# nanoporetech/bonito

Hardware: AMD Instinct MI355X
Metric: signal samples/sec/GPU (chunk=10000, batch=512) + read accuracy vs ref (higher is better)
Workload: dtype f16

## Files before the change

### bonito_amd/_lib.py

```python
import ctypes as C
import os

_HERE = os.path.dirname(os.path.abspath(__file__))
LIB_PATH = os.environ.get("BONITO_HIP_LIB") or os.path.join(_HERE, "libbonito_hip.so")


class HipEngineError(RuntimeError):
    """An entry point of libbonito_hip.so reported an error."""


class bh_layer_t(C.Structure):
    _fields_ = [
        ("kind", C.c_int32), ("in_size", C.c_int32), ("out_size", C.c_int32),
        ("winlen", C.c_int32), ("stride", C.c_int32), ("padding", C.c_int32),
        ("activation", C.c_int32), ("reverse", C.c_int32),
        ("nhead", C.c_int32), ("dim_ff", C.c_int32), ("win_left", C.c_int32), ("win_right", C.c_int32),
        ("scale_factor", C.c_int32), ("groups", C.c_int32), ("add_residual", C.c_int32), ("quantize", C.c_int32), ("reserved_i", C.c_int32 * 1),
        ("scale", C.c_float), ("clamp_lo", C.c_float), ("clamp_hi", C.c_float),
        ("blank_score", C.c_float), ("alpha", C.c_float), ("eps", C.c_float), ("reserved_f", C.c_float * 2),
        ("w0", C.c_void_p), ("b0", C.c_void_p), ("w1", C.c_void_p), ("b1", C.c_void_p),
        ("w2", C.c_void_p), ("w3", C.c_void_p), ("w4", C.c_void_p), ("w5", C.c_void_p),
    ]


# ... 20 lines not shown
    "bh_encoder_ack": (_i, [_vp, _l]),
    "bh_encoder_describe": (_i, [_vp, C.c_char_p, _sz]),
    "bh_encoder_profile": (_i, [_vp, _i]),
    "bh_encoder_profile_read": (_i, [_vp, C.POINTER(C.c_float), C.POINTER(_i)]),
    "bh_crf_viterbi_workspace": (_sz, [_i, _i, _i]),
    "bh_crf_viterbi": (_i, [_vp, _i, _i, _i, _i, _f, _l, _l, _vp, _vp, _vp, _vp, _vp]),
    "bh_crf_reverse_complement": (_i, [_vp, _vp, _i, _i, _i, _i, _l, _l, _vp]),
    "bh_crf_logz": (_i, [_vp, _i, _i, _i, _f, _vp, _vp, _vp]),
    "bh_crf_seq_workspace": (_sz, [_i, _i, _i, _i]),
    "bh_crf_seq_logz": (_i, [_vp, _i, _i, _i, _i, _f, _l, _l, _vp, _i, _i, _vp, _vp, _vp, _vp]),
    "bh_crf_seq_viterbi": (_i, [_vp, _i, _i, _i, _i, _f, _l, _l, _vp, _i, _i, _vp, _vp, _vp, _vp, _vp]),
    "bh_crf_seq_logz_free": (_i, [_vp, _i, _i, _i, _f, _l, _l, _vp, _i, _i, _vp, _vp, _vp, _vp]),
    "bh_crf_logz_dense": (_i, [_vp, _i, _i, _i, _i, _f, _l, _l, _vp, _vp]),
    "bh_sw_workspace": (_sz, [_i, _i, _i]),
    "bh_sw_align": (_i, [_vp, _l, _vp, _vp, _l, _vp, _i, _i, _i, _i, _i, _vp, _sz, _vp, _vp, _l, _vp, _vp]),
    "bh_set_option": (_i, [C.c_char_p, _i]),
    "bh_signal_normalise": (_i, [_vp, _vp, _vp, _vp, _i, _i, C.c_double, C.c_double, C.c_double, C.c_double, C.c_double, C.c_double,
                            _i, _vp, _vp, _vp, _vp, _vp]),
    "bh_signal_chunks": (_i, [_vp, _vp, _vp, _vp, _vp, _vp, _vp, _vp, _vp, _vp, _i, _i, _vp, _vp]),
    "bh_crf_posterior_viterbi_workspace": (_sz, [_i, _i, _i]),
    "bh_crf_posterior_viterbi": (_i, [_vp, _i, _i, _i, _f, _vp, _vp, _vp, _vp]),
    "bh_beam_search_workspace": (_sz, [_i, _i, _i]),
    "bh_beam_search": (_i, [_vp, _i, _i, _i, _i, _f, _f, _f, _f, _vp, _vp, _vp, _vp, _vp, _vp]),
    "bh_linear": (_i, [_vp, _vp, _vp, _vp, _i, _i, _i, _i, _i, _i, _i, _f, _f, _f, _i, _i, _l, _l, _i, _vp]),
    "bh_conv1d_first": (_i, [_vp, _vp, _vp, _vp, _i, _i, _i, _i, _i, _i, _i, _f, _f, _l, _l, _vp]),
    "bh_conv1d_packed_halves": (_sz, [_i, _i, _i]),
    "bh_conv1d_pack": (_i, [_vp, _i, _i, _i, _vp]),
    "bh_conv1d": (_i, [_vp, _vp, _vp, _vp, _i, _i, _i, _i, _i, _i, _i, _i, _f, _f, _l, _l, _vp]),
    "bh_ctc_greedy_decode": (_i, [_vp, _vp, _i, _i, _f, _f, _vp, _vp, _vp, _vp, _vp]),
    "bh_ctc_beam_search_workspace": (_sz, [_l, _i, _i, _i]),
    "bh_ctc_beam_search": (_i, [_vp, _vp, _i, _i, _i, _f, _vp, _vp, _vp, _vp, _vp]),
    "bh_dwconv1d": (_i, [_vp, _vp, _vp, _i, _i, _i, _i, _i, _i, _vp]),
    "bh_rotary_table": (_i, [_i, _i, _vp]),
    "bh_attention": (_i, [_vp, _vp, _vp, _i, _i, _i, _i, _i, _i, _vp]),
    "bh_attention_prerotated": (_i, [_vp, _vp, _i, _i, _i, _i, _i, _i, _vp]),
    "bh_rmsnorm_residual": (_i, [_vp, _vp, _vp, _vp, _l, _i, _f, _f, _vp]),
    "bh_lstm_pack_whh": (_i, [_vp, _i, _vp]),
    "bh_host_compact": (_l, [_vp, _l, _vp]),
    "bh_host_chunk_rows": (_l, [_vp, _l, _i, _i, _l, _l, _vp]),
    "bh_host_format_read": (_l, [_vp, _vp, _vp, _vp, _i, _l, _l, _i, _i, _i, _i, _i, _i, C.c_double, C.c_char_p, C.c_char_p, _l, _l,
                                 _vp, _l, _vp, _vp]),
    "bh_host_mean_qscore": (C.c_double, [C.c_char_p, _l]),
    "bh_host_svb16_decode": (_l, [_vp, _l, _l, _vp]),
    "bh_lstm_workspace": (_sz, [_i, _i]),
    "bh_lstm_layer": (_i, [_vp, _vp, _vp, _i, _i, _i, _i, _vp, _vp, _i, _vp]),
    "bh_lstm_q8_layer": (_i, [_vp, _f, _vp, _vp, _vp, _i, _i, _i, _i, _i, _vp, _vp, _vp, _vp]),
# ... 47 lines not shown
```

### bonito_amd/csrc/beam.hip

```cpp
#include <stdlib.h>

#include "common.h"
#include "kernels.h"
#include <cstring>
#include "../../include/bh_lse_table.h"

namespace bh {

__device__ const float g_lse_tab[BH_LSE_TABLE_SIZE] = {BH_LSE_TABLE_VALUES};

__device__ __forceinline__ float lse2_tab(float a, float b, const float* tab) {
    float m = fmaxf(a, b);
    float d = fabsf(a - b);
    if (!(d < BH_LSE_RANGE)) return m;
    float x = d * BH_LSE_SCALE;
    int i = (int)x;
    float f = x - (float)i;
    float t0 = tab[i];
    float sp = __fmaf_rn(f, tab[i + 1] - t0, t0);
    return m + sp;
}

__device__ __forceinline__ float lse2_tab_nb(float a, float b, const float* tab) {
    const float m = fmaxf(a, b);
// ... 222 lines not shown
                res_m[t - tlo] = (int8_t)(k != 0);
                res_p[t - tlo] = (int8_t)(k != 0 ? 1 + (st & 3) : 0);
                if (k != 0) st = (k - 1) * q + (st >> 2);
            }
            s_state[0] = st;
        }
        __syncthreads();
        for (int i = threadIdx.x; i < thi - tlo; i += blockDim.x) { mo[tlo + i] = res_m[i]; pth[tlo + i] = res_p[i]; }
        __syncthreads();
    }
}

struct BeamArgs {
    const half_t* scores;
    const float* beta;
    int N, T, S, state_len, W;
    float blank, cut;
    uint8_t* bp;
    int* final_slot;
    long long* dbg;
    float inv_bin;
    float* P;
    int nt;
};

template <int STATE_LEN>
__host__ __device__ constexpr int beam_btb() {
#ifdef BH_BTB
    return BH_BTB;
#else
    return STATE_LEN >= 4 ? 1 : 2;
#endif
}
constexpr int MAXW = 32;

__device__ __forceinline__ unsigned bs_hash0(int s) { return ((unsigned)s + 1u) * 2654435761u; }
__device__ __forceinline__ unsigned bs_mix(unsigned h, int x) {
    h = (h ^ ((unsigned)x + 1u)) * 16777619u;
    return h ^ (h >> 15);
}
__device__ __forceinline__ unsigned bs_ukey(float k) {
    unsigned u = __float_as_uint(k);
    return (u & 0x80000000u) ? ~u : (u | 0x80000000u);
}
__device__ __forceinline__ int popc64(unsigned long long m) { return __popcll(m); }
__device__ __forceinline__ unsigned long long lanemask_lt(int lane) { return (1ull << lane) - 1ull; }
// ... 170 lines not shown
constexpr unsigned TAG_MASK = 0x1ffffu;

struct BeamTable {
    int* cnt;
    uint2_t* ent;
    int* ov_cnt;
    uint2_t* ov;
};

__device__ __forceinline__ unsigned bucket_match(const uint4_t& e0, unsigned hash, unsigned want) {
    unsigned d = 32u;
    d = min(d, e0.x == hash ? e0.y - want : 32u);
    d = min(d, e0.z == hash ? e0.w - want : 32u);
    return d;
}

__device__ __forceinline__ void dma16(const char* g, char* lds) {
    const unsigned l = (unsigned)__builtin_amdgcn_readfirstlane((int)(unsigned)(size_t)(__attribute__((address_space(3))) char*)lds);
    asm volatile("s_mov_b32 m0, %0\n\ts_nop 0\n\tglobal_load_lds_dwordx4 %1, off" ::"s"(l), "v"(g) : "memory");
}
__device__ __forceinline__ void dma16_nt(const char* g, char* lds) {
    const unsigned l = (unsigned)__builtin_amdgcn_readfirstlane((int)(unsigned)(size_t)(__attribute__((address_space(3))) char*)lds);
    asm volatile("s_mov_b32 m0, %0\n\ts_nop 0\n\tglobal_load_lds_dwordx4 %1, off nt" ::"s"(l), "v"(g) : "memory");
}

#include "../../include/bh_bs2.h"
typedef float float2_t __attribute__((ext_vector_type(2)));

__device__ __forceinline__ float2_t fma2(float2_t a, float2_t b, float2_t c) { return __builtin_elementwise_fma(a, b, c); }
__device__ __forceinline__ float2_t splat2(float v) { return float2_t{v, v}; }

__device__ __forceinline__ float2_t bs2_exp2(float2_t x) {
    x.x = __builtin_amdgcn_fmed3f(x.x, -BH_BS2_XMAX, BH_BS2_XMAX);
    x.y = __builtin_amdgcn_fmed3f(x.y, -BH_BS2_XMAX, BH_BS2_XMAX);
    const float2_t t = fma2(x, splat2(BH_BS2_LOG2E), splat2(BH_BS2_MAGIC));
    const float2_t n = t - splat2(BH_BS2_MAGIC);
    const float2_t f = fma2(x, splat2(BH_BS2_LOG2E), -n);
    float2_t p = splat2(BH_BS2_E5);
    p = fma2(p, f, splat2(BH_BS2_E4));
    p = fma2(p, f, splat2(BH_BS2_E3));
    p = fma2(p, f, splat2(BH_BS2_E2));
    p = fma2(p, f, splat2(BH_BS2_E1));
    p = fma2(p, f, splat2(BH_BS2_E0));
    float2_t r;
    r.x = __uint_as_float(__float_as_uint(p.x) + (__float_as_uint(t.x) << 23));
    r.y = __uint_as_float(__float_as_uint(p.y) + (__float_as_uint(t.y) << 23));
// ... 370 lines not shown
                    Pn[(long)t * 4 + m_raw] = (m_raw == 0 ? c4[0] : m_raw == 1 ? c4[1] : m_raw == 2 ? c4[2] : c4[3]) / tot;
                }
            } else {
                if (act) *(float4_t*)(an + 4 * m) = o;
                const float inv = 1.0f / ((cls[0] + cls[1]) + (cls[2] + cls[3]));
                if (lane < 4 && live) Pn[(long)t * 4 + lane] = (lane == 0 ? cls[0] : lane == 1 ? cls[1] : lane == 2 ? cls[2] : cls[3]) * inv;
            }
            cur ^= 1;
        }
    }
}

template <int STATE_LEN, int CPW, bool FUSE>
__host__ __device__ constexpr int beam_scan_waves() { return !FUSE ? 0 : (1 << (2 * STATE_LEN)) / 4 >= 64 ? CPW : 1; }

template <int STATE_LEN, int CPW, bool DBG, bool FUSE = false>
__global__ __launch_bounds__(64 * (CPW + beam_scan_waves<STATE_LEN, CPW, FUSE>())) __attribute__((amdgpu_waves_per_eu(1, 8))) void beam_kernel(BeamArgs p) {
    extern __shared__ __attribute__((aligned(16))) char smem[];
    constexpr int S = 1 << (2 * STATE_LEN);
    constexpr int sh = 2 * (STATE_LEN - 1);
    constexpr int BTB = beam_btb<STATE_LEN>();
    constexpr int QS = S / 4, GLS = QS < 64 ? QS : 64;
    constexpr int NTHR = 64 * (CPW + beam_scan_waves<STATE_LEN, CPW, FUSE>());
    static_assert(!FUSE || QS >= 64 || CPW * QS <= 64, "one scan wave must hold the chunks of the workgroup");
    static_assert(NBK == HBINS, "the selection histogram reuses the bucket fill counters");
    static_assert(beam_wave_lds<STATE_LEN>() % 16 == 0 && BEAM_TAB_LDS % 16 == 0, "LDS regions must stay 16-byte aligned");
    const int T = p.T, W = p.W;
    const int lane = threadIdx.x & 63;
    const int wave_all = __builtin_amdgcn_readfirstlane(threadIdx.x >> 6);
    const bool scan_role = FUSE && wave_all >= CPW;
    const int slot_raw = !scan_role ? wave_all : QS >= 64 ? wave_all - CPW : lane / GLS;
    const bool slot_ok = slot_raw < CPW && blockIdx.x * CPW + slot_raw < p.N;
    const int wave = slot_ok ? slot_raw : 0;
    const int n = blockIdx.x * CPW + wave;
    float* tab = (float*)smem;
    for (int i = threadIdx.x; i < BH_LSE_TABLE_SIZE; i += NTHR) tab[i] = g_lse_tab[i];
    __syncthreads();
    if (!slot_ok && (!scan_role || QS >= 64)) return;
    char* mine = smem + BEAM_TAB_LDS + wave * beam_wave_lds<STATE_LEN>();
    half_t* st_sc = (half_t*)mine;
    float* st_b = (float*)(st_sc + 2 * BTB * 4 * S);
    constexpr int SCAN_LDS = scan_wave_lds<STATE_LEN>();
    char* scan_mem = smem + BEAM_TAB_LDS + CPW * beam_wave_lds<STATE_LEN>() + wave * SCAN_LDS;
    if (scan_role) {
        float* al = (float*)scan_mem;
        const int sm = QS >= 64 ? lane : lane - (lane / GLS) * GLS;
        if (slot_ok) *(float4_t*)(al + 4 * sm) = float4_t{1.0f, 1.0f, 1.0f, 1.0f};
        const float ebl = __expf(__builtin_amdgcn_fmed3f(p.blank, -BH_BS2_XMAX, BH_BS2_XMAX));
        float* Pn = p.P + (long)n * T * 4;
        int cb = 0;
        for (int tb0 = 0, blk = 0; tb0 < T; tb0 += BTB, ++blk) {
            const int nsteps = min(BTB, T - tb0);
            __syncthreads();
            const half_t* blk_sc = st_sc + (blk & 1) * BTB * 4 * S;
            const float* blk_b = st_b + (blk & 1) * BTB * S;
            for (int u = 0; u < nsteps; ++u) {
                scan_step<STATE_LEN>(ebl, blk_sc + u * 4 * S, blk_b + u * S, al + cb * S, al + (cb ^ 1) * S, sm, slot_ok, Pn + (long)(tb0 + u) * 4);
                cb ^= 1;
            }
        }
        return;
    }
    BeamTable tb;
    tb.ent = (uint2_t*)(st_b + 2 * BTB * S);
    uint4_t* b_elem = (uint4_t*)(tb.ent + NBK * BKE);
    uint2_t* m_pair = (uint2_t*)(b_elem + MAXW);
    tb.ov = m_pair + MAXW;
    tb.cnt = (int*)(tb.ov + MAXW);
    tb.ov_cnt = tb.cnt + NBK;
    int* hist = tb.cnt;
    uint8_t* st_bp = (uint8_t*)(tb.ov_cnt + 4);

    const half_t* sc = p.scores + (long)n * T * 4 * S;
    const float* bn = p.beta + (long)n * (T + 1) * S;
    uint8_t* bpn = p.bp + (long)n * T * MAXW;

    long long dsec[6] = {0, 0, 0, 0, 0, 0};
    const int ce[3] = {lane & (MAXW - 1), lane >> 2, 16 + (lane >> 2)};
    const int mx = lane & 3;
    const bool stay_lane = lane < MAXW;

    int nb;
#pragma unroll
    for (int i = 0; i < NBK * BKE / 64; ++i) tb.ent[lane + 64 * i] = uint2_t{0u, 0xffffffffu};
    if (lane < MAXW) tb.ov[lane] = uint2_t{0u, 0xffffffffu};
    *(uint4_t*)(tb.cnt + 4 * lane) = uint4_t{0u, 0u, 0u, 0u};
    if (lane < 4) tb.ov_cnt[lane] = 0;
    if (lane < MAXW) m_pair[lane] = uint2_t{0u, 0xffffffffu};
    if (lane < MAXW) b_elem[lane] = uint4_t{0u, 0u, 0u, 0u};
    {
        const int per = (S + 63) / 64;
        unsigned prefix = 0u;
        const int want = W < S ? W : S;
        for (int bit = 31; bit >= 0; --bit) {
            const unsigned trial = prefix | (1u << bit);
            int cnt = 0;
            for (int i = 0; i < per; ++i) {
// ... 8 lines not shown
            const int s = i * 64 + lane;
            const unsigned u = s < S ? bs_ukey(bn[s]) : 0u;
            n_gt += popc64(__ballot(u > prefix));
        }
        const int need = want - n_gt;
        int tie_before = 0, before = 0;
        for (int i = 0; i < per; ++i) {
            const int s = i * 64 + lane;
            const unsigned u = s < S ? bs_ukey(bn[s]) : 0u;
            const unsigned long long eq = __ballot(s < S && u == prefix);
            const bool tie_ok = ((eq >> lane) & 1ull) && (tie_before + popc64(eq & lanemask_lt(lane))) < need;
            const bool take = (s < S && u > prefix) || tie_ok;
            const unsigned long long tm = __ballot(take);
            if (take) {
                const int slot = before + popc64(tm & lanemask_lt(lane));
                b_elem[slot] = uint4_t{(unsigned)s, bs_hash0(s), 0u , 0u};
            }
            tie_before += popc64(eq);
            before += popc64(tm);
        }
        nb = before;
    }

    auto dma_rows = [&](const char* src, char* dst, int n16) {
        for (int i0 = 0; i0 < n16; i0 += 64)
            if (i0 + lane < n16) { if (p.nt) dma16_nt(src + (long)(i0 + lane) * 16, dst + i0 * 16); else dma16(src + (long)(i0 + lane) * 16, dst + i0 * 16); }
    };
    auto stage = [&](int tb0, int which) {
        const int nsteps = min(BTB, T - tb0);
        dma_rows((const char*)(sc + (long)tb0 * 4 * S), (char*)(st_sc + which * BTB * 4 * S), nsteps * S / 2);
        dma_rows((const char*)(bn + (long)(tb0 + 1) * S), (char*)(st_b + which * BTB * S), nsteps * S / 4);
    };
    if (T > 0) stage(0, 0);
    for (int tb0 = 0, blk = 0; tb0 < T; tb0 += BTB, ++blk) {
        const int nsteps = min(BTB, T - tb0);
        {
            long long ts0 = 0;
            if (DBG) ts0 = __builtin_readcyclecounter();
            asm volatile("s_waitcnt vmcnt(0)" ::: "memory");
            if (FUSE) __syncthreads();
            if (DBG) dsec[5] += __builtin_readcyclecounter() - ts0;
            if (tb0 + BTB < T) stage(tb0 + BTB, (blk + 1) & 1);
        }
        const half_t* blk_sc = st_sc + (blk & 1) * BTB * 4 * S;
        const float* blk_b = st_b + (blk & 1) * BTB * S;
        for (int u = 0; u < nsteps; ++u) {
            const half_t* row = blk_sc + u * 4 * S;
            const float* b1 = blk_b + u * S;
            const unsigned tag = ((unsigned)(tb0 + u) & TAG_MASK) << 15;
            long long tc0 = 0;
            if (DBG) tc0 = __builtin_readcyclecounter();
            float cs[3];
            unsigned ch[3];
            int cst[3], cinfo[3];
            uint4_t el[3];
#pragma unroll
            for (int i = 0; i < 3; ++i) el[i] = b_elem[ce[i]];
            float mv[3], bg[3];
            uint4_t ent0[3];
            {
                const int es = (int)(el[0].x & (unsigned)(S - 1));
                cst[0] = es; ch[0] = el[0].y; cinfo[0] = ce[0];
                bg[0] = b1[es];
                if (stay_lane && ce[0] < nb) {
                    const int bk = (int)(ch[0] & (NBK - 1));
                    const int pos = atomicAdd(&tb.cnt[bk], 1);
                    const uint2_t e{ch[0], tag | ((unsigned)es << 5) | (unsigned)lane};
                    if (pos < BKE) tb.ent[bk * BKE + pos] = e;
                    else tb.ov[atomicAdd(tb.ov_cnt, 1)] = e;
                }
            }
#pragma unroll
            for (int i = 1; i < 3; ++i) {
                const int es = (int)(el[i].x & (unsigned)(S - 1));
                const int s2 = ((es << 2) | mx) & (S - 1);
                cst[i] = s2;
                ch[i] = bs_mix(el[i].y, mx);
                cinfo[i] = ce[i] | (1 << 5) | (mx << 6);
                mv[i] = (float)row[s2 * 4 + (es >> sh)];
                bg[i] = b1[s2];
                ent0[i] = *(const uint4_t*)(tb.ent + (int)(ch[i] & (NBK - 1)) * BKE);
            }
            const int n_ov = tb.ov_cnt[0];
            cs[0] = (stay_lane && ce[0] < nb) ? __uint_as_float(el[0].z) + p.blank : -INFINITY;
            unsigned dhit[3];
#pragma unroll
            for (int i = 1; i < 3; ++i) {
                cs[i] = ce[i] < nb ? __uint_as_float(el[i].z) + mv[i] : -INFINITY;
                dhit[i] = bucket_match(ent0[i], ch[i], tag | ((unsigned)cst[i] << 5));
            }
            if (n_ov > 0) {
                for (int k = 0; k < n_ov; ++k) {
                    const uint2_t e = tb.ov[k];
#pragma unroll
                    for (int i = 1; i < 3; ++i)
                        dhit[i] = min(dhit[i], e.x == ch[i] ? e.y - (tag | ((unsigned)cst[i] << 5)) : 32u);
                }
            }
#pragma unroll
            for (int i = 1; i < 3; ++i)
                if (ce[i] < nb && dhit[i] < 32u) {
                    m_pair[dhit[i]] = uint2_t{__float_as_uint(cs[i]), (unsigned)cinfo[i]};
                    cs[i] = -INFINITY;
                }
            *(uint4_t*)(tb.cnt + 4 * lane) = uint4_t{0u, 0u, 0u, 0u};
// ... 212 lines not shown
    const int threads = S < 64 ? 64 : S;
    {
        int b_threads = 0;
        size_t b_lds = 0;
        backward_geometry(S, N, sa.cpb, b_threads, b_lds);
        if (b_lds > 64 * 1024) BH_CHECK_HIP(bh_max_lds((const void*)crf_backward_kernel, (int)b_lds));
        hipLaunchKernelGGL(crf_backward_kernel, dim3((N + sa.cpb - 1) / sa.cpb), dim3(b_threads), b_lds, stream, sa);
        sa.cpb = 1;
    }
    PostVitArgs pa{sa, bp, moves, path};
    int TB = (32 * 1024) / S; if (TB > 512) TB = 512; if (TB < 1) TB = 1;
    const size_t lds_pv = (size_t)(BH_LSE_TABLE_SIZE + 2 + 4 * S + 4) * sizeof(float) + (size_t)TB * S + 2 * TB + 32;
    hipLaunchKernelGGL(crf_posterior_viterbi_kernel, dim3(N), dim3(threads), lds_pv, stream, pa);
    BH_CHECK_HIP(hipGetLastError());
    return 0;
}

namespace {
struct SideStream { hipStream_t stream = nullptr; hipEvent_t fork = nullptr, join = nullptr; };
int g_beam_select = 0;
int g_beam_fork = -1;
int g_beam_cpw = 0;
int g_beam_fuse = -1;
SideStream* side_stream(int S) {
    if (g_beam_fork == 0 || (g_beam_fork < 0 && S > 64 && S < 1024)) return nullptr;
    thread_local SideStream per_dev[16];
    int dev = 0;
    if (hipGetDevice(&dev) != hipSuccess || dev < 0 || dev >= 16) return nullptr;
    SideStream& s = per_dev[dev];
    if (!s.stream) {
        if (hipStreamCreateWithFlags(&s.stream, hipStreamNonBlocking) != hipSuccess) { s.stream = nullptr; return nullptr; }
        if (hipEventCreateWithFlags(&s.fork, hipEventDisableTiming) != hipSuccess ||
            hipEventCreateWithFlags(&s.join, hipEventDisableTiming) != hipSuccess) return nullptr;
    }
    return &s;
}
}

int bh_k_beam_search(const void* scores, int N, int T, int state_len, int beam_width, float beam_cut,
                     float blank, float q_scale, float q_offset, void* workspace, int8_t* sequence,
                     int8_t* qstring, int8_t* moves, float* qfloat, hipStream_t stream) {
    using namespace bh;
    BH_REQUIRE(state_len >= 1 && state_len <= 5, "beam_search: state_len must be in 1..5 (got %d)", state_len);
    BH_REQUIRE(N > 0 && T > 0, "beam_search: empty problem N=%d T=%d", N, T);
    BH_REQUIRE(beam_width >= 1 && beam_width <= 32, "beam_search: beam_width must be in 1..32 (got %d)", beam_width);
    BH_REQUIRE(beam_cut >= 1.0f, "beam_search: beam_cut must be >= 1");
    BH_REQUIRE(T < (1 << 17), "beam_search: at most 131071 steps per chunk (got %d)", T);
    int S = 1;
    for (int i = 0; i < state_len; ++i) S *= 4;
    auto align = [](size_t x) { return (x + 255) / 256 * 256; };
    char* w = (char*)workspace;
    float* beta = (float*)w;   w += align((size_t)N * (T + 1) * S * sizeof(float));
    w += align((size_t)N * (T + 1) * sizeof(double));
    w += align((size_t)N * sizeof(double));
    float* P = (float*)w;      w += align((size_t)N * T * 4 * sizeof(float));
    uint8_t* bp = (uint8_t*)w; w += align((size_t)N * T * 32);
    int* fin = (int*)w;         w += align((size_t)N * sizeof(int));
    long long* dbg = getenv("BH_BEAM_DEBUG") ? (long long*)w : nullptr;

    const bool fuse = g_beam_fuse != 0 && S <= 256;
    {
        Bs2Args a2{(const half_t*)scores, beta, N, T, blank, g_decode_nt};
        auto launch_bwd = [&](auto kern, int cpb, size_t lds, int threads) -> int {
            if (lds > 64 * 1024) BH_CHECK_HIP(bh_max_lds((const void*)kern, (int)lds));
            hipLaunchKernelGGL(kern, dim3((N + cpb - 1) / cpb), dim3(threads), lds, stream, a2);
            return 0;
        };
        int rc = -2;
        switch (state_len) {
            case 1: rc = launch_bwd(bs2_backward_kernel<1>, Bs2Geo<1>::CPB, (size_t)Bs2Geo<1>::UPB * Bs2Geo<1>::UNIT_LDS, Bs2Geo<1>::UPB * Bs2Geo<1>::UT); break;
            case 2: rc = launch_bwd(bs2_backward_kernel<2>, Bs2Geo<2>::CPB, (size_t)Bs2Geo<2>::UPB * Bs2Geo<2>::UNIT_LDS, Bs2Geo<2>::UPB * Bs2Geo<2>::UT); break;
            case 3: rc = launch_bwd(bs2_backward_kernel<3>, Bs2Geo<3>::CPB, (size_t)Bs2Geo<3>::UPB * Bs2Geo<3>::UNIT_LDS, Bs2Geo<3>::UPB * Bs2Geo<3>::UT); break;
            case 4: rc = launch_bwd(bs2_backward_kernel<4>, Bs2Geo<4>::CPB, (size_t)Bs2Geo<4>::UPB * Bs2Geo<4>::UNIT_LDS, Bs2Geo<4>::UPB * Bs2Geo<4>::UT); break;
            case 5: rc = launch_bwd(bs2_backward_kernel<5>, Bs2Geo<5>::CPB, (size_t)Bs2Geo<5>::UPB * Bs2Geo<5>::UNIT_LDS, Bs2Geo<5>::UPB * Bs2Geo<5>::UT); break;
        }
        if (rc) return rc;
    }
    SideStream* side = fuse ? nullptr : side_stream(S);
    const bool fork = side != nullptr;
    if (fork) {
        BH_CHECK_HIP(hipEventRecord(side->fork, stream));
        BH_CHECK_HIP(hipStreamWaitEvent(side->stream, side->fork, 0));
    }
    if (!fuse) {
        Bs2FwdArgs f2{(const half_t*)scores, beta, P, N, T, blank, g_decode_nt};
        hipStream_t fs = fork ? side->stream : stream;
        auto launch_fwd = [&](auto kern, int cpb, size_t chunk_lds) -> int {
            const size_t lds = (size_t)cpb * chunk_lds;
            if (lds > 64 * 1024) BH_CHECK_HIP(bh_max_lds((const void*)kern, (int)lds));
            hipLaunchKernelGGL(kern, dim3((N + cpb - 1) / cpb), dim3(256), lds, fs, f2);
            return 0;
        };
        int rc = -2;
        switch (state_len) {
            case 1: rc = launch_fwd(bs2_forward_post_kernel<1>, Bs2FwdGeo<1>::CPB, Bs2FwdGeo<1>::CHUNK_LDS); break;
            case 2: rc = launch_fwd(bs2_forward_post_kernel<2>, Bs2FwdGeo<2>::CPB, Bs2FwdGeo<2>::CHUNK_LDS); break;
            case 3: rc = launch_fwd(bs2_forward_post_kernel<3>, Bs2FwdGeo<3>::CPB, Bs2FwdGeo<3>::CHUNK_LDS); break;
            case 4: rc = launch_fwd(bs2_forward_post_kernel<4>, Bs2FwdGeo<4>::CPB, Bs2FwdGeo<4>::CHUNK_LDS); break;
            case 5: rc = launch_fwd(bs2_forward_post_kernel<5>, Bs2FwdGeo<5>::CPB, Bs2FwdGeo<5>::CHUNK_LDS); break;
        }
        if (rc) return rc;
    }
    if (fork) BH_CHECK_HIP(hipEventRecord(side->join, side->stream));
    BeamArgs ba{(const half_t*)scores, beta, N, T, S, state_len, beam_width, blank, logf(beam_cut), bp, fin, dbg,
                g_beam_select ? 0.0f : 256.0f / fmaxf(logf(beam_cut), 1e-6f), P, g_decode_nt};
    auto launch_beam = [&](auto kern, int cpw, size_t wave_lds, size_t scan_lds = 0) -> int {
        const size_t lds_beam = (size_t)BEAM_TAB_LDS + cpw * (wave_lds + scan_lds);
        if (lds_beam > 64 * 1024)
            BH_CHECK_HIP(bh_max_lds((const void*)kern, (int)lds_beam));
        hipLaunchKernelGGL(kern, dim3((N + cpw - 1) / cpw), dim3(64 * (cpw + (!scan_lds ? 0 : S >= 256 ? cpw : 1))), lds_beam, stream, ba);
        return 0;
    };
    int lrc = -2;
    int cpw4 = g_beam_cpw;
    if (fuse && state_len == 4 && cpw4 <= 0) {
        const long cus = bh_cu_count();
        cpw4 = (long)N <= 5 * cus ? 1 : (long)N <= 6 * cus ? 2 : 4;
    }
    if (false) {
    } else if (fuse && state_len == 4 && !dbg && cpw4 == 4) {
        lrc = launch_beam(beam_kernel<4, 4, false, true>, 4, beam_wave_lds<4>(), scan_wave_lds<4>());
    } else if (fuse && state_len == 4 && !dbg && cpw4 == 2) {
        lrc = launch_beam(beam_kernel<4, 2, false, true>, 2, beam_wave_lds<4>(), scan_wave_lds<4>());
    } else if (fuse) {
        switch (state_len * 2 + (dbg ? 1 : 0)) {
            case 2: lrc = launch_beam(beam_kernel<1, 4, false, true>, 4, beam_wave_lds<1>(), scan_wave_lds<1>()); break;
            case 3: lrc = launch_beam(beam_kernel<1, 4, true, true>, 4, beam_wave_lds<1>(), scan_wave_lds<1>()); break;
            case 4: lrc = launch_beam(beam_kernel<2, 4, false, true>, 4, beam_wave_lds<2>(), scan_wave_lds<2>()); break;
            case 5: lrc = launch_beam(beam_kernel<2, 4, true, true>, 4, beam_wave_lds<2>(), scan_wave_lds<2>()); break;
            case 6: lrc = launch_beam(beam_kernel<3, 4, false, true>, 4, beam_wave_lds<3>(), scan_wave_lds<3>()); break;
            case 7: lrc = launch_beam(beam_kernel<3, 4, true, true>, 4, beam_wave_lds<3>(), scan_wave_lds<3>()); break;
            case 8: lrc = launch_beam(beam_kernel<4, 1, false, true>, 1, beam_wave_lds<4>(), scan_wave_lds<4>()); break;
            case 9: lrc = launch_beam(beam_kernel<4, 1, true, true>, 1, beam_wave_lds<4>(), scan_wave_lds<4>()); break;
        }
    } else
    switch (state_len * 2 + (dbg ? 1 : 0)) {
        case 2: lrc = launch_beam(beam_kernel<1, 4, false>, 4, beam_wave_lds<1>()); break;
        case 3: lrc = launch_beam(beam_kernel<1, 4, true>, 4, beam_wave_lds<1>()); break;
        case 4: lrc = launch_beam(beam_kernel<2, 4, false>, 4, beam_wave_lds<2>()); break;
        case 5: lrc = launch_beam(beam_kernel<2, 4, true>, 4, beam_wave_lds<2>()); break;
        case 6: lrc = launch_beam(beam_kernel<3, 4, false>, 4, beam_wave_lds<3>()); break;
        case 7: lrc = launch_beam(beam_kernel<3, 4, true>, 4, beam_wave_lds<3>()); break;
        case 8: lrc = launch_beam(beam_kernel<4, 1, false>, 1, beam_wave_lds<4>()); break;
        case 9: lrc = launch_beam(beam_kernel<4, 1, true>, 1, beam_wave_lds<4>()); break;
        case 10: lrc = launch_beam(beam_kernel<5, 1, false>, 1, beam_wave_lds<5>()); break;
        case 11: lrc = launch_beam(beam_kernel<5, 1, true>, 1, beam_wave_lds<5>()); break;
    }
    if (lrc) return lrc;
    if (fork) BH_CHECK_HIP(hipStreamWaitEvent(stream, side->join, 0));
    FinArgs fa{bp, fin, P, N, T, q_scale, q_offset, sequence, qstring, moves, qfloat};
    hipLaunchKernelGGL(beam_finalize_kernel, dim3(N), dim3(64), 0, stream, fa);
    BH_CHECK_HIP(hipGetLastError());
    return 0;
}

int bh_k_decode_set_option(const char* name, int value) {
    if (name && !strcmp(name, "beam_fork")) { g_beam_fork = value; return 0; }
    if (name && !strcmp(name, "beam_select")) { g_beam_select = value; return 0; }
    if (name && !strcmp(name, "beam_fuse")) { g_beam_fuse = value; return 0; }
    if (name && !strcmp(name, "beam_cpw")) { g_beam_cpw = value; return 0; }
    if (name && !strcmp(name, "decode_nt")) { g_decode_nt = value; return 0; }
    if (name && !strcmp(name, "viterbi_quad")) { bh::g_viterbi_quad = value; return 0; }
    return 1;
}
```

### bonito_amd/csrc/engine.cpp

```cpp
#include <hip/hip_runtime.h>
#include <stdarg.h>
#include <stdio.h>
#include <string.h>

#include <algorithm>
#include <atomic>
#include <cmath>
#include <string>
#include <vector>

#include "../../include/bonito_hip.h"
#include "common.h"
#include "kernels.h"

static thread_local char g_err[1024] = "";
void bh_set_error(const char* fmt, ...) {
    va_list ap;
    va_start(ap, fmt);
    vsnprintf(g_err, sizeof(g_err), fmt, ap);
    va_end(ap);
}
extern "C" const char* bh_last_error(void) { return g_err; }
extern "C" int bh_abi_version(void) { return BH_ABI_VERSION; }
extern "C" size_t bh_sizeof_layer(void) { return sizeof(bh_layer_t); }
// ... 1318 lines not shown
}

extern "C" int bh_encoder_debug_read(bh_encoder_t* e, void* host, size_t bytes, size_t offset) {
    BH_REQUIRE(e && host && offset + bytes <= e->lstm_ws.bytes, "encoder_debug_read: out of range");
    BH_CHECK_HIP(hipMemcpy(host, (char*)e->lstm_ws.p + offset, bytes, hipMemcpyDeviceToHost));
    return 0;
}
extern "C" int bh_encoder_set_option(bh_encoder_t* e, const char* name, int value) {
    BH_REQUIRE(e && name, "encoder_set_option: null argument");
    if (!strcmp(name, "lstm_force_slow")) { e->lstm_force_slow = (e->lstm_force_slow & ~1) | (value & 1); return 0; }
    if (!strcmp(name, "lstm_fused")) { e->lstm_fused = value; return 0; }
    if (!strcmp(name, "attn_ring")) { e->attn_ring = value; return 0; }
    if (!strcmp(name, "lstm_wide")) { e->lstm_wide = value; return 0; }
    if (!strcmp(name, "lstm_prefill")) { e->lstm_prefill = value; return 0; }
    if (!strcmp(name, "lstm_q8")) { e->lstm_q8 = value; return 0; }
    if (!strcmp(name, "lstm_exchange")) { e->lstm_exchange = value; return 0; }
    if (!strcmp(name, "lstm_pair")) { e->lstm_pair = value; return 0; }
    if (!strcmp(name, "norm_fuse")) { e->norm_fuse = value; return 0; }
    if (!strcmp(name, "gemm_v1")) { bh_k_linear_force_v1(value); return 0; }
    if (!strcmp(name, "lstm_tune")) { e->lstm_force_slow = (e->lstm_force_slow & 1) | (value << 8); return 0; }
    BH_REQUIRE(false, "encoder_set_option: unknown option '%s'", name);
}
extern "C" size_t bh_beam_search_workspace(int N, int T, int state_len) { return bh_k_beam_workspace(N, T, state_len); }
extern "C" int bh_beam_search(const void* scores, int N, int T, int state_len, int beam_width, float beam_cut,
                              float blank_score, float q_scale, float q_offset, void* workspace, int8_t* sequence,
                              int8_t* qstring, int8_t* moves, float* qfloat, void* stream) {
    BH_REQUIRE(scores && workspace && sequence && qstring && moves, "beam_search: null pointer");
    return bh_k_beam_search(scores, N, T, state_len, beam_width, beam_cut, blank_score, q_scale, q_offset, workspace,
                            sequence, qstring, moves, qfloat, (hipStream_t)stream);
}
extern "C" int bh_crf_reverse_complement(const void* in, void* out, int N, int T, int state_len, int layout_5s,
                                         long stride_n, long stride_t, void* stream) {
    BH_REQUIRE(in && out, "crf_reverse_complement: null pointer");
    return bh_k_crf_revcomp(in, out, N, T, state_len, layout_5s, stride_n, stride_t, (hipStream_t)stream);
}
extern "C" int bh_crf_logz(const void* scores, int N, int T, int state_len, float blank_score, void* workspace,
                           double* logz, void* stream) {
    BH_REQUIRE(scores && workspace && logz, "crf_logz: null pointer");
    return bh_k_crf_logz(scores, N, T, state_len, blank_score, workspace, logz, (hipStream_t)stream);
}
extern "C" size_t bh_crf_seq_workspace(int N, int T, int Lmax, int state_len) {
    return bh_k_crf_seq_workspace(N, T, Lmax, state_len);
}
extern "C" int bh_crf_seq_logz(const void* scores, int N, int T, int state_len, int layout_5s, float blank_score, long stride_n,
                               long stride_t, const void* targets, int Lmax, int target_bytes, const int32_t* target_lengths,
                               void* workspace, float* logz_out, void* stream) {
// ... 84 lines not shown
```

### bonito_amd/csrc/kernels.h

```cpp
#pragma once
#include <hip/hip_runtime.h>
#include <stdint.h>

int bh_k_linear(const void* X, const void* W, const float* bias, void* out, int M, int N, int K,
                int ldx, int ldw, int ldo, int act, float scale, float clamp_lo, float clamp_hi,
                int gated, int row_div, long row_s_hi, long row_s_lo, int row_lim, hipStream_t stream,
                const void* residual = nullptr, int ldres = 0, float res_scale = 1.0f);

void bh_k_linear_force_v1(int on);
void bh_k_linear_stagger(int units);
void bh_k_linear_order(int order);
void bh_k_linear_gf(int gf);
void bh_k_linear_tile16(int on);

int bh_k_conv_first(const void* signal, const float* w, const float* bias, void* out, int N, int Lin,
                    int Lout, int Cout, int K, int stride, int pad, int act, float clamp_lo,
                    float clamp_hi, long os_n, long os_t, hipStream_t stream);
int bh_k_conv_igemm(const void* in, const void* wpk, const float* bias, void* out, int N, int Lin,
                    int Lout, int Cin, int Cout, int K, int stride, int pad, int act, float clamp_lo,
                    float clamp_hi, long os_n, long os_t, hipStream_t stream);

int bh_k_lstm_layer(const void* gates_in, const void* whh_packed, void* h_out, int T, int N, int H,
                    int reverse, int* err_flag, hipStream_t stream, int n_rings, int* xcc_ws, int force_slow);
size_t bh_k_lstm_ws_bytes(int N, int H);
// ... 34 lines not shown
                   hipStream_t stream);
int bh_k_beam_search(const void* scores, int N, int T, int state_len, int beam_width, float beam_cut,
                     float blank, float q_scale, float q_offset, void* workspace, int8_t* sequence,
                     int8_t* qstring, int8_t* moves, float* qfloat, hipStream_t stream);

int bh_k_attention(const void* qkv, void* out, const float* cos_sin, int N, int T, int nhead, int head_dim,
                   int win_left, int win_right, hipStream_t stream);
int bh_k_rmsnorm_residual(const void* a, const void* x, const float* w, void* out, long M, int D, float alpha,
                          float eps, hipStream_t stream);

int bh_k_dwconv(const void* in, const float* w, void* out, int N, int Lin, int Lout, int C, int K, int stride,
                int pad, hipStream_t stream);
int bh_k_ctc_head(const void* in, const float* w, const float* bias, void* out, long M, int features, int classes,
                  hipStream_t stream);
int bh_k_ctc_greedy(const float* logp, const long* offs, int R, int C, float qscale, float qbias, int8_t* seq,
                    int8_t* qual, int* path, int* count, hipStream_t stream);
size_t bh_k_ctc_beam_workspace(long total_steps, int R, int C, int beam_size);
int bh_k_ctc_prefix_beam(const float* logp, const long* offs, int R, int C, int beam_size, float threshold, void* workspace,
                         int8_t* labels, int* path, int* count, hipStream_t stream);
size_t bh_k_posterior_viterbi_workspace(int N, int T, int state_len);
int bh_k_posterior_viterbi(const void* scores, int N, int T, int state_len, float blank, void* workspace, int8_t* moves,
                           int8_t* path, hipStream_t stream);
int bh_k_decode_set_option(const char* name, int value);
namespace bh { extern int g_viterbi_quad; }
int bh_k_conv_set_option(const char* name, int value);
int bh_k_conv_front3_ok(int c1_eff, int K1, int s1, int c2_in_eff, int c2_eff, int K2, int s2, int c3_in_eff, int c3_out, int K3, int s3);
int bh_k_conv_front3(const void* signal, int N, int L0, const float* w1, const float* b1, int K1, int pad1, int act1, float lo1, float hi1,
                     const void* w2pk, const float* b2, int K2, int pad2, int act2, float lo2, float hi2, const void* w3pk,
                     const float* b3, int Cout3, int K3, int stride3, int pad3, int act3, float lo3, float hi3, void* out, long os_n,
                     long os_t, hipStream_t stream);
int bh_k_linear_qkv_rotary(const void* X, const void* W, const float* bias, void* out, int M, int D, int K, const float* cos_sin,
                           int T, float qscale, hipStream_t stream);
int bh_k_attention_prerotated(const void* qkv, void* out, int N, int T, int nhead, int head_dim, int win_left, int win_right,
                              hipStream_t stream);
inline bool bh_k_attention_ring_serves(int win_left, int win_right) {
    return win_left >= 0 && win_right >= 0 && win_left <= 128 && win_right <= 144;
}
int bh_k_signal_normalise(const int16_t* raw, const long* offs, const float* cal_scale, const float* cal_offset, int R,
                          int strategy, double qa, double qb, double shift_mult, double scale_mult, double fixed_shift,
                          double fixed_scale, int do_trim, double* shift, double* scale, int* weak, int* trim, hipStream_t stream);
int bh_k_signal_chunks(const int16_t* raw, const long* offs, const float* cal_scale, const float* cal_offset, const double* shift,
                       const double* scale, const int* weak, const int* chunk_read, const long* chunk_start, const long* chunk_len,
                       int n_chunks, int L, void* out, hipStream_t stream);
int bh_k_lstm_wide_ok(int H);
int bh_k_lstm_layer_wide(const void* gates_perm, const void* whh_tiles, void* h_out, int T, int N, int H, int reverse,
                         int* err_flag, hipStream_t stream, int n_rings, int* xcc_ws, int force_slow, void* ex = nullptr, int R = 0,
// ... 20 lines not shown
```

### include/bonito_hip.h

```cpp
#ifndef BONITO_HIP_H
#define BONITO_HIP_H

#include <stddef.h>
#include <stdint.h>

#ifdef __cplusplus
extern "C" {
#endif

#define BH_ABI_VERSION 1

enum { BH_ACT_NONE = 0, BH_ACT_SWISH = 1, BH_ACT_TANH = 2, BH_ACT_RELU = 3 };

enum {
    BH_LAYER_CONV = 1,
    BH_LAYER_LSTM = 2,
    BH_LAYER_LINEAR_CRF = 3,
    BH_LAYER_CLAMP = 4,
    BH_LAYER_TRANSFORMER = 5,
    BH_LAYER_UPSAMPLE = 6,
    BH_LAYER_TCS_BLOCK = 7,
    BH_LAYER_CTC_DECODER = 8,
    BH_LAYER_DWCONV = 9,
    BH_LAYER_RESIDUAL_PROJ = 10,
// ... 86 lines not shown
                size_t workspace_bytes, int32_t* result, uint32_t* ops, long ops_stride, int32_t* n_ops, void* stream);

int bh_signal_normalise(const int16_t* raw, const long* offsets, const float* cal_scale, const float* cal_offset, int n_reads,
                        int strategy, double quantile_a, double quantile_b, double shift_mult, double scale_mult,
                        double fixed_shift, double fixed_scale, int do_trim, double* shift, double* scale, int* weak, int* trim,
                        void* stream);
int bh_signal_chunks(const int16_t* raw, const long* offsets, const float* cal_scale, const float* cal_offset,
                     const double* shift, const double* scale, const int* weak, const int* chunk_read, const long* chunk_start,
                     const long* chunk_len, int n_chunks, int chunk_samples, void* out, void* stream);

int bh_lstm_q8_layer(const void* x, float bound, const float* w_ih, const float* w_hh, const float* bias, int T, int N, int H,
                     int reverse, int variant, void* h16_out, int8_t* hq_frag, int32_t* sums, void* stream);

int bh_set_option(const char* name, int value);

size_t bh_crf_posterior_viterbi_workspace(int N, int T, int state_len);
int bh_crf_posterior_viterbi(const void* scores, int N, int T, int state_len, float blank_score, void* workspace,
                             int8_t* moves, int8_t* path, void* stream);

size_t bh_beam_search_workspace(int N, int T, int state_len);
int bh_beam_search(const void* scores, int N, int T, int state_len, int beam_width, float beam_cut,
                   float blank_score, float q_scale, float q_offset, void* workspace, int8_t* sequence,
                   int8_t* qstring, int8_t* moves, float* qfloat, void* stream);

int bh_linear(const void* X, const void* W, const float* bias, void* out, int M, int N, int K, int ldx,
              int ldw, int ldo, int act, float scale, float clamp_lo, float clamp_hi, int gated,
              int row_div, long row_s_hi, long row_s_lo, int row_lim, void* stream);
int bh_conv1d_first(const void* signal, const float* w, const float* bias, void* out, int N, int Lin,
                    int Cout, int K, int stride, int pad, int act, float clamp_lo, float clamp_hi,
                    long os_n, long os_t, void* stream);
size_t bh_conv1d_packed_halves(int Cin, int Cout, int K);
int bh_conv1d_pack(const float* w, int Cin, int Cout, int K, uint16_t* packed);
int bh_conv1d(const void* in, const void* wpacked, const float* bias, void* out, int N, int Lin, int Cin,
              int Cout, int K, int stride, int pad, int act, float clamp_lo, float clamp_hi, long os_n,
              long os_t, void* stream);
int bh_ctc_greedy_decode(const float* logp, const long* offsets, int R, int classes, float qscale, float qbias,
                         int8_t* labels, int8_t* qual, int* path, int* count, void* stream);
size_t bh_ctc_beam_search_workspace(long total_steps, int R, int classes, int beam_size);
int bh_ctc_beam_search(const float* logp, const long* offsets, int R, int classes, int beam_size, float threshold,
                       void* workspace, int8_t* labels, int* path, int* count, void* stream);
int bh_dwconv1d(const void* in, const float* w, void* out, int N, int Lin, int C, int K, int stride, int pad,
                void* stream);
int bh_rotary_table(int T, int dim, float* out);
int bh_attention(const void* qkv, void* out, const float* cos_sin, int N, int T, int nhead, int head_dim,
                 int win_left, int win_right, void* stream);
int bh_attention_prerotated(const void* qkv, void* out, int N, int T, int nhead, int head_dim, int win_left, int win_right, void* stream);
// ... 21 lines not shown
```

Before: 343.4 million.

## Replace workgroup barriers with per-wave LDS flag handoff between scan and beam waves

In the fused beam-search kernel, each scan wave now stages its chunk's score and beta blocks itself and signals the paired beam wave through LDS counters (landed/consumed). This replaces the workgroup-wide __syncthreads per block. Waves from different chunks no longer stall each other, and the DMA for the next block is issued early. In exchange the code adds spin-wait polling with a timeout bound, a pinned host error word, and timeout reporting and LDS-query entry points. It also relies on a hand-written memory-ordering protocol, which risks races or hangs.

```diff
diff --git a/bonito_amd/_lib.py b/bonito_amd/_lib.py
--- a/bonito_amd/_lib.py
+++ b/bonito_amd/_lib.py
@@ -66,6 +66,8 @@
     "bh_crf_posterior_viterbi": (_i, [_vp, _i, _i, _i, _f, _vp, _vp, _vp, _vp]),
     "bh_beam_search_workspace": (_sz, [_i, _i, _i]),
     "bh_beam_search": (_i, [_vp, _i, _i, _i, _i, _f, _f, _f, _f, _vp, _vp, _vp, _vp, _vp, _vp]),
+    "bh_beam_search_error": (_i, [C.POINTER(_i), C.POINTER(_i), C.POINTER(_i)]),
+    "bh_beam_search_lds": (_i, [_i, _i, C.POINTER(_i), C.POINTER(_i)]),
     "bh_linear": (_i, [_vp, _vp, _vp, _vp, _i, _i, _i, _i, _i, _i, _i, _f, _f, _f, _i, _i, _l, _l, _i, _vp]),
     "bh_conv1d_first": (_i, [_vp, _vp, _vp, _vp, _i, _i, _i, _i, _i, _i, _i, _f, _f, _l, _l, _vp]),
     "bh_conv1d_packed_halves": (_sz, [_i, _i, _i]),
diff --git a/bonito_amd/csrc/beam.hip b/bonito_amd/csrc/beam.hip
--- a/bonito_amd/csrc/beam.hip
+++ b/bonito_amd/csrc/beam.hip
@@ -268,6 +268,8 @@
     float inv_bin;
     float* P;
     int nt;
+    unsigned max_spins;
+    int* err;
 };
 
 template <int STATE_LEN>
@@ -484,6 +486,31 @@
 __device__ __forceinline__ void dma16_nt(const char* g, char* lds) {
     const unsigned l = (unsigned)__builtin_amdgcn_readfirstlane((int)(unsigned)(size_t)(__attribute__((address_space(3))) char*)lds);
     asm volatile("s_mov_b32 m0, %0\n\ts_nop 0\n\tglobal_load_lds_dwordx4 %1, off nt" ::"s"(l), "v"(g) : "memory");
+}
+
+__device__ __forceinline__ void seq_post(int* w, int v) {
+    const unsigned a = (unsigned)(size_t)(__attribute__((address_space(3))) int*)w;
+    asm volatile("ds_write_b32 %0, %1" ::"v"(a), "v"(v) : "memory");
+}
+__device__ __forceinline__ int seq_peek(const int* w) {
+    const unsigned a = (unsigned)(size_t)(__attribute__((address_space(3))) const int*)w;
+    int v;
+    asm volatile("ds_read_b32 %0, %1\n\ts_waitcnt lgkmcnt(0)" : "=v"(v) : "v"(a) : "memory");
+    return __builtin_amdgcn_readfirstlane(v);
+}
+__device__ __forceinline__ bool seq_wait(const int* w, int need, unsigned max_spins) {
+    for (unsigned spin = 0;; ++spin) {
+        if (seq_peek(w) >= need) return true;
+        if (spin >= max_spins) return false;
+        __builtin_amdgcn_s_sleep(1);
+    }
+}
+__device__ __forceinline__ void seq_timeout(int* err, int lane, int n, int blk, int role) {
+    if (lane == 0 && err) {
+        err[1] = n; err[2] = blk; err[3] = role;
+        __threadfence_system();
+        err[0] = 1;
+    }
 }
 
 #include "../../include/bh_bs2.h"
@@ -900,6 +927,7 @@
     constexpr int BTB = beam_btb<STATE_LEN>();
     constexpr int QS = S / 4, GLS = QS < 64 ? QS : 64;
     constexpr int NTHR = 64 * (CPW + beam_scan_waves<STATE_LEN, CPW, FUSE>());
+    constexpr bool PAIR = FUSE && QS >= 64;
     static_assert(!FUSE || QS >= 64 || CPW * QS <= 64, "one scan wave must hold the chunks of the workgroup");
     static_assert(NBK == HBINS, "the selection histogram reuses the bucket fill counters");
     static_assert(beam_wave_lds<STATE_LEN>() % 16 == 0 && BEAM_TAB_LDS % 16 == 0, "LDS regions must stay 16-byte aligned");
@@ -913,13 +941,30 @@
     const int n = blockIdx.x * CPW + wave;
     float* tab = (float*)smem;
     for (int i = threadIdx.x; i < BH_LSE_TABLE_SIZE; i += NTHR) tab[i] = g_lse_tab[i];
+    constexpr int SCAN_LDS = scan_wave_lds<STATE_LEN>();
+    if (PAIR && !scan_role && lane == 0) {
+        int* w0 = (int*)(smem + BEAM_TAB_LDS + CPW * beam_wave_lds<STATE_LEN>() + wave_all * SCAN_LDS + 2 * S * 4);
+        w0[0] = -1; w0[8] = -1;
+    }
     __syncthreads();
     if (!slot_ok && (!scan_role || QS >= 64)) return;
     char* mine = smem + BEAM_TAB_LDS + wave * beam_wave_lds<STATE_LEN>();
     half_t* st_sc = (half_t*)mine;
     float* st_b = (float*)(st_sc + 2 * BTB * 4 * S);
-    constexpr int SCAN_LDS = scan_wave_lds<STATE_LEN>();
     char* scan_mem = smem + BEAM_TAB_LDS + CPW * beam_wave_lds<STATE_LEN>() + wave * SCAN_LDS;
+    int* landed = (int*)(scan_mem + 2 * S * 4);
+    int* consumed = landed + 8;
+    const half_t* sc = p.scores + (long)n * T * 4 * S;
+    const float* bn = p.beta + (long)n * (T + 1) * S;
+    auto dma_rows = [&](const char* src, char* dst, int n16) {
+        for (int i0 = 0; i0 < n16; i0 += 64)
+            if (i0 + lane < n16) { if (p.nt) dma16_nt(src + (long)(i0 + lane) * 16, dst + i0 * 16); else dma16(src + (long)(i0 + lane) * 16, dst + i0 * 16); }
+    };
+    auto stage = [&](int tb0, int which) {
+        const int nsteps = min(BTB, T - tb0);
+        dma_rows((const char*)(sc + (long)tb0 * 4 * S), (char*)(st_sc + which * BTB * 4 * S), nsteps * S / 2);
+        dma_rows((const char*)(bn + (long)(tb0 + 1) * S), (char*)(st_b + which * BTB * S), nsteps * S / 4);
+    };
     if (scan_role) {
         float* al = (float*)scan_mem;
         const int sm = QS >= 64 ? lane : lane - (lane / GLS) * GLS;
@@ -927,16 +972,33 @@
         const float ebl = __expf(__builtin_amdgcn_fmed3f(p.blank, -BH_BS2_XMAX, BH_BS2_XMAX));
         float* Pn = p.P + (long)n * T * 4;
         int cb = 0;
+        long long ssec[2] = {0, 0};
+        bool lost = false;
+        if (PAIR && T > 0) stage(0, 0);
         for (int tb0 = 0, blk = 0; tb0 < T; tb0 += BTB, ++blk) {
             const int nsteps = min(BTB, T - tb0);
-            __syncthreads();
+            long long ts0 = 0;
+            if (DBG) ts0 = __builtin_readcyclecounter();
+            if (PAIR) {
+                asm volatile("s_waitcnt vmcnt(0)" ::: "memory");
+                seq_post(landed, blk);
+                if (tb0 + BTB < T) {
+                    if (!lost && !seq_wait(consumed, blk - 1, p.max_spins)) { lost = true; seq_timeout(p.err, lane, n, blk, 1); }
+                    stage(tb0 + BTB, (blk + 1) & 1);
+                }
+            } else {
+                __syncthreads();
+            }
+            if (DBG) { const long long t1 = __builtin_readcyclecounter(); ssec[1] += t1 - ts0; ts0 = t1; }
             const half_t* blk_sc = st_sc + (blk & 1) * BTB * 4 * S;
             const float* blk_b = st_b + (blk & 1) * BTB * S;
             for (int u = 0; u < nsteps; ++u) {
                 scan_step<STATE_LEN>(ebl, blk_sc + u * 4 * S, blk_b + u * S, al + cb * S, al + (cb ^ 1) * S, sm, slot_ok, Pn + (long)(tb0 + u) * 4);
                 cb ^= 1;
             }
-        }
+            if (DBG) ssec[0] += __builtin_readcyclecounter() - ts0;
+        }
+        if (DBG && PAIR && lane == 0) { p.dbg[(long)n * 8 + 6] = ssec[0]; p.dbg[(long)n * 8 + 7] = ssec[1]; }
         return;
     }
     BeamTable tb;
@@ -949,8 +1011,6 @@
     int* hist = tb.cnt;
     uint8_t* st_bp = (uint8_t*)(tb.ov_cnt + 4);
 
-    const half_t* sc = p.scores + (long)n * T * 4 * S;
-    const float* bn = p.beta + (long)n * (T + 1) * S;
     uint8_t* bpn = p.bp + (long)n * T * MAXW;
 
     long long dsec[6] = {0, 0, 0, 0, 0, 0};
@@ -1005,25 +1065,21 @@
         nb = before;
     }
 
-    auto dma_rows = [&](const char* src, char* dst, int n16) {
-        for (int i0 = 0; i0 < n16; i0 += 64)
-            if (i0 + lane < n16) { if (p.nt) dma16_nt(src + (long)(i0 + lane) * 16, dst + i0 * 16); else dma16(src + (long)(i0 + lane) * 16, dst + i0 * 16); }
-    };
-    auto stage = [&](int tb0, int which) {
-        const int nsteps = min(BTB, T - tb0);
-        dma_rows((const char*)(sc + (long)tb0 * 4 * S), (char*)(st_sc + which * BTB * 4 * S), nsteps * S / 2);
-        dma_rows((const char*)(bn + (long)(tb0 + 1) * S), (char*)(st_b + which * BTB * S), nsteps * S / 4);
-    };
-    if (T > 0) stage(0, 0);
+    bool lost = false;
+    if (!PAIR && T > 0) stage(0, 0);
     for (int tb0 = 0, blk = 0; tb0 < T; tb0 += BTB, ++blk) {
         const int nsteps = min(BTB, T - tb0);
         {
             long long ts0 = 0;
             if (DBG) ts0 = __builtin_readcyclecounter();
-            asm volatile("s_waitcnt vmcnt(0)" ::: "memory");
-            if (FUSE) __syncthreads();
+            if (PAIR) {
+                if (!lost && !seq_wait(landed, blk, p.max_spins)) { lost = true; seq_timeout(p.err, lane, n, blk, 0); }
+            } else {
+                asm volatile("s_waitcnt vmcnt(0)" ::: "memory");
+                if (FUSE) __syncthreads();
+            }
             if (DBG) dsec[5] += __builtin_readcyclecounter() - ts0;
-            if (tb0 + BTB < T) stage(tb0 + BTB, (blk + 1) & 1);
+            if (!PAIR && tb0 + BTB < T) stage(tb0 + BTB, (blk + 1) & 1);
         }
         const half_t* blk_sc = st_sc + (blk & 1) * BTB * 4 * S;
         const float* blk_b = st_b + (blk & 1) * BTB * S;
@@ -1064,6 +1120,7 @@
                 bg[i] = b1[s2];
                 ent0[i] = *(const uint4_t*)(tb.ent + (int)(ch[i] & (NBK - 1)) * BKE);
             }
+            if (PAIR && u == nsteps - 1) seq_post(consumed, blk);
             const int n_ov = tb.ov_cnt[0];
             cs[0] = (stay_lane && ce[0] < nb) ? __uint_as_float(el[0].z) + p.blank : -INFINITY;
             unsigned dhit[3];
@@ -1322,6 +1379,17 @@
 int g_beam_fork = -1;
 int g_beam_cpw = 0;
 int g_beam_fuse = -1;
+unsigned g_beam_max_spins = 1000000u;
+int* g_beam_err = nullptr;
+int* beam_err_words() {
+    if (!g_beam_err) {
+        int* e = nullptr;
+        if (hipHostMalloc((void**)&e, 4 * sizeof(int), hipHostMallocPortable) != hipSuccess) return nullptr;
+        e[0] = e[1] = e[2] = e[3] = 0;
+        g_beam_err = e;
+    }
+    return g_beam_err;
+}
 SideStream* side_stream(int S) {
     if (g_beam_fork == 0 || (g_beam_fork < 0 && S > 64 && S < 1024)) return nullptr;
     thread_local SideStream per_dev[16];
@@ -1335,6 +1403,41 @@
     }
     return &s;
 }
+}
+
+int bh_k_beam_search_error(int* chunk, int* block, int* role) {
+    volatile int* e = g_beam_err;
+    if (!e || !e[0]) return 0;
+    const int n = e[1], b = e[2], r = e[3];
+    e[0] = 0;
+    if (chunk) *chunk = n;
+    if (block) *block = b;
+    if (role) *role = r;
+    bh_set_error("beam_search: the %s wave of chunk %d timed out waiting for block %d (hand-off poll bound %u); the output of that call is invalid",
+                 r ? "scan" : "beam", n, b, g_beam_max_spins);
+    return 1;
+}
+
+int bh_k_beam_lds(int state_len, int cpw, int* workgroup_lds, int* workgroups_per_cu) {
+    using namespace bh;
+    BH_REQUIRE(state_len >= 1 && state_len <= 5 && workgroup_lds && workgroups_per_cu, "beam_lds: bad arguments");
+    const bool fuse = g_beam_fuse != 0 && state_len <= 4;
+    size_t wave = 0, scan = 0;
+    switch (state_len) {
+        case 1: wave = beam_wave_lds<1>(); scan = scan_wave_lds<1>(); break;
+        case 2: wave = beam_wave_lds<2>(); scan = scan_wave_lds<2>(); break;
+        case 3: wave = beam_wave_lds<3>(); scan = scan_wave_lds<3>(); break;
+        case 4: wave = beam_wave_lds<4>(); scan = scan_wave_lds<4>(); break;
+        case 5: wave = beam_wave_lds<5>(); break;
+    }
+    int c = state_len >= 4 ? 1 : 4, per_cu = 1;
+    if (fuse && state_len == 4) {
+        c = cpw == 1 || cpw == 2 ? cpw : 4;
+        per_cu = c == 1 ? 5 : c == 2 ? 3 : 2;
+    }
+    *workgroup_lds = (int)(BEAM_TAB_LDS + c * (wave + (fuse ? scan : 0)));
+    *workgroups_per_cu = per_cu;
+    return 0;
 }
 
 int bh_k_beam_search(const void* scores, int N, int T, int state_len, int beam_width, float beam_cut,
@@ -1359,6 +1462,12 @@
     long long* dbg = getenv("BH_BEAM_DEBUG") ? (long long*)w : nullptr;
 
     const bool fuse = g_beam_fuse != 0 && S <= 256;
+    int* err = nullptr;
+    if (fuse && S == 256) {
+        err = beam_err_words();
+        BH_REQUIRE(err != nullptr, "beam_search: no pinned memory for the error words");
+        if (bh_k_beam_search_error(nullptr, nullptr, nullptr)) return 1;
+    }
     {
         Bs2Args a2{(const half_t*)scores, beta, N, T, blank, g_decode_nt};
         auto launch_bwd = [&](auto kern, int cpb, size_t lds, int threads) -> int {
@@ -1403,7 +1512,7 @@
     }
     if (fork) BH_CHECK_HIP(hipEventRecord(side->join, side->stream));
     BeamArgs ba{(const half_t*)scores, beta, N, T, S, state_len, beam_width, blank, logf(beam_cut), bp, fin, dbg,
-                g_beam_select ? 0.0f : 256.0f / fmaxf(logf(beam_cut), 1e-6f), P, g_decode_nt};
+                g_beam_select ? 0.0f : 256.0f / fmaxf(logf(beam_cut), 1e-6f), P, g_decode_nt, g_beam_max_spins, err};
     auto launch_beam = [&](auto kern, int cpw, size_t wave_lds, size_t scan_lds = 0) -> int {
         const size_t lds_beam = (size_t)BEAM_TAB_LDS + cpw * (wave_lds + scan_lds);
         if (lds_beam > 64 * 1024)
@@ -1418,8 +1527,9 @@
         cpw4 = (long)N <= 5 * cus ? 1 : (long)N <= 6 * cus ? 2 : 4;
     }
     if (false) {
-    } else if (fuse && state_len == 4 && !dbg && cpw4 == 4) {
-        lrc = launch_beam(beam_kernel<4, 4, false, true>, 4, beam_wave_lds<4>(), scan_wave_lds<4>());
+    } else if (fuse && state_len == 4 && cpw4 == 4) {
+        lrc = dbg ? launch_beam(beam_kernel<4, 4, true, true>, 4, beam_wave_lds<4>(), scan_wave_lds<4>())
+                  : launch_beam(beam_kernel<4, 4, false, true>, 4, beam_wave_lds<4>(), scan_wave_lds<4>());
     } else if (fuse && state_len == 4 && !dbg && cpw4 == 2) {
         lrc = launch_beam(beam_kernel<4, 2, false, true>, 2, beam_wave_lds<4>(), scan_wave_lds<4>());
     } else if (fuse) {
@@ -1459,6 +1569,7 @@
     if (name && !strcmp(name, "beam_select")) { g_beam_select = value; return 0; }
     if (name && !strcmp(name, "beam_fuse")) { g_beam_fuse = value; return 0; }
     if (name && !strcmp(name, "beam_cpw")) { g_beam_cpw = value; return 0; }
+    if (name && !strcmp(name, "beam_max_spins")) { g_beam_max_spins = value >= 0 ? (unsigned)value : 1000000u; return 0; }
     if (name && !strcmp(name, "decode_nt")) { g_decode_nt = value; return 0; }
     if (name && !strcmp(name, "viterbi_quad")) { bh::g_viterbi_quad = value; return 0; }
     return 1;
diff --git a/bonito_amd/csrc/engine.cpp b/bonito_amd/csrc/engine.cpp
--- a/bonito_amd/csrc/engine.cpp
+++ b/bonito_amd/csrc/engine.cpp
@@ -1364,6 +1364,10 @@
     BH_REQUIRE(false, "encoder_set_option: unknown option '%s'", name);
 }
 extern "C" size_t bh_beam_search_workspace(int N, int T, int state_len) { return bh_k_beam_workspace(N, T, state_len); }
+extern "C" int bh_beam_search_error(int* chunk, int* block, int* role) { return bh_k_beam_search_error(chunk, block, role); }
+extern "C" int bh_beam_search_lds(int state_len, int cpw, int* workgroup_lds, int* workgroups_per_cu) {
+    return bh_k_beam_lds(state_len, cpw, workgroup_lds, workgroups_per_cu);
+}
 extern "C" int bh_beam_search(const void* scores, int N, int T, int state_len, int beam_width, float beam_cut,
                               float blank_score, float q_scale, float q_offset, void* workspace, int8_t* sequence,
                               int8_t* qstring, int8_t* moves, float* qfloat, void* stream) {
diff --git a/bonito_amd/csrc/kernels.h b/bonito_amd/csrc/kernels.h
--- a/bonito_amd/csrc/kernels.h
+++ b/bonito_amd/csrc/kernels.h
@@ -80,6 +80,8 @@
 int bh_k_posterior_viterbi(const void* scores, int N, int T, int state_len, float blank, void* workspace, int8_t* moves,
                            int8_t* path, hipStream_t stream);
 int bh_k_decode_set_option(const char* name, int value);
+int bh_k_beam_search_error(int* chunk, int* block, int* role);
+int bh_k_beam_lds(int state_len, int cpw, int* workgroup_lds, int* workgroups_per_cu);
 namespace bh { extern int g_viterbi_quad; }
 int bh_k_conv_set_option(const char* name, int value);
 int bh_k_conv_front3_ok(int c1_eff, int K1, int s1, int c2_in_eff, int c2_eff, int K2, int s2, int c3_in_eff, int c3_out, int K3, int s3);
diff --git a/include/bonito_hip.h b/include/bonito_hip.h
--- a/include/bonito_hip.h
+++ b/include/bonito_hip.h
@@ -132,6 +132,8 @@
 int bh_beam_search(const void* scores, int N, int T, int state_len, int beam_width, float beam_cut,
                    float blank_score, float q_scale, float q_offset, void* workspace, int8_t* sequence,
                    int8_t* qstring, int8_t* moves, float* qfloat, void* stream);
+int bh_beam_search_error(int* chunk, int* block, int* role);
+int bh_beam_search_lds(int state_len, int cpw, int* workgroup_lds, int* workgroups_per_cu);
 
 int bh_linear(const void* X, const void* W, const float* bias, void* out, int M, int N, int K, int ldx,
               int ldw, int ldo, int act, float scale, float clamp_lo, float clamp_hi, int gated,
```

Result: no change. 344.6 million (median of 6 runs) (+0.3%).
